# kevalmorabia97/CoVA-Web-Object-Detection

Hardware: AMD Instinct MI355X
Metric: webpages/sec fwd+bwd (90 bboxes, K=24) (higher is better)
Workload: dtype f32

## Files before the change

### cova-web-object-detection_amd/csrc/conv_wgrad4.hip

```cpp
#include "mma.h"
#include "options.h"
#include <type_traits>

#ifndef WG4_ABL
#define WG4_ABL 0
#endif

#if defined(__HIP_DEVICE_COMPILE__) && !defined(__gfx950__)
#error "conv_wgrad4.hip is written for gfx950 (160 KB of LDS per workgroup)"
#endif

#ifdef WG4_TRACE
__device__ unsigned long long g_wg4_trace[2 * 4 * 8];
#define WG4_STAMP(slot)                                                                                         \
    do {                                                                                                        \
        if (blockIdx.x == 0 && (wave == 0 || wave == 4) && wg4_k >= 100 && wg4_k < 104 && lane == 0)           \
            g_wg4_trace[((wave >> 2) * 4 + (wg4_k - 100)) * 8 + (slot)] = __builtin_amdgcn_s_memtime();         \
    } while (0)
#else
#define WG4_STAMP(slot) do { } while (0)
#endif

namespace {

namespace wg4 {
constexpr int THREADS = 512;
constexpr int ROW = 10;
constexpr int TILE_FLOATS = 128 * ROW + 32;
constexpr int BUF_FLOATS = 2 * 4 * TILE_FLOATS;
constexpr int RAW_FLOATS = 36 * 64;
constexpr int PART_FLOATS = 9 * 4096;
}

struct Wg4Args {
    const float *act, *dz, *dz2;
    float *part;
    const float *act_abc, *dz_abc;
    float *dz_out;
    int act_relu;
    int H, W, tiles_y, strips, nseg_y, seg_rows, nsegs;
};

__device__ __forceinline__ void wg4_bt6(const float (&d)[6], float (&o)[6])
{
    const float a = fmaf(-4.f, d[2], d[4]), b = fmaf(-4.f, d[1], d[3]);
    const float c = d[4] - d[2], e = 2.f * (d[3] - d[1]);
    o[0] = fmaf(4.f, d[0], fmaf(-5.f, d[2], d[4]));
    o[1] = a + b;
    o[2] = a - b;
    o[3] = c + e;
    o[4] = c - e;
    o[5] = fmaf(4.f, d[1], fmaf(-5.f, d[3], d[5]));
}

__device__ __forceinline__ void wg4_a6(const float (&g)[4], float (&o)[6])
{
    const float p = g[0] + g[2], q = g[1] + g[3];
    const float u = fmaf(4.f, g[2], g[0]), w = 2.f * fmaf(4.f, g[3], g[1]);
    o[0] = g[0];
    o[1] = p + q;
    o[2] = p - q;
    o[3] = u + w;
    o[4] = u - w;
    o[5] = g[3];
}

template <int HALF>
__device__ __forceinline__ void wg4_bt_half(float d0, float d1, float d2, float d3, float d4, float d5, float (&o)[3])
{
    if (HALF == 0) {
        const float a = fmaf(-4.f, d2, d4), b = fmaf(-4.f, d1, d3);
        o[0] = fmaf(4.f, d0, fmaf(-5.f, d2, d4));
        o[1] = a + b;
        o[2] = a - b;
    } else {
        const float c = d4 - d2, e = 2.f * (d3 - d1);
        o[0] = fmaf(4.f, d1, fmaf(-5.f, d3, d5));
        o[1] = c + e;
        o[2] = c - e;
    }
}

template <int HALF>
__device__ __forceinline__ void wg4_a_half(float g0, float g1, float g2, float g3, float (&o)[3])
{
    if (HALF == 0) {
        const float p = g0 + g2, q = g1 + g3;
        o[0] = g0;
        o[1] = p + q;
        o[2] = p - q;
    } else {
        const float u = fmaf(4.f, g2, g0), w = 2.f * fmaf(4.f, g3, g1);
        o[0] = g3;
        o[1] = u + w;
        o[2] = u - w;
    }
}

struct Wg4It {
    int seg, rr, nrows, b, strip, ty;
};

template <bool PROA, int PROD>
__global__ __launch_bounds__(wg4::THREADS, 1) void conv3x3_wgrad4_kernel(const Wg4Args a)
{
    using namespace wg4;
    __shared__ __attribute__((aligned(16))) float s_op[2 * BUF_FLOATS];
    __shared__ __attribute__((aligned(1024))) float s_raw[8 * RAW_FLOATS];
    const int tid = threadIdx.x, lane = tid & 63;
    const int wave = __builtin_amdgcn_readfirstlane(tid >> 6);
    const int H = a.H, W = a.W;
    const int G = (int)gridDim.x, NW = G >> 1;
    int half, walker;
    if ((G & 15) == 0) {
        const int m = (int)blockIdx.x >> 3, x = (int)blockIdx.x & 7;
        half = m & 1;
        walker = (m >> 1) * 8 + x;
    } else {
        half = (int)blockIdx.x & 1;
        walker = (int)blockIdx.x >> 1;
    }
    const bool vrole = wave < 4;
    const int tcol = wave & 3;
    const int pg = wave & 1, cp = (wave >> 1) & 1, np = wave >> 2;
    const int l15 = lane & 15, kq = lane >> 4;

    int n_k = 0;
    for (int s = walker; s < a.nsegs; s += NW) n_k += min(a.seg_rows, a.tiles_y - (s % a.nseg_y) * a.seg_rows);

    auto seg_setup = [&](Wg4It &it) __attribute__((always_inline)) {
        const int s = it.seg < a.nsegs ? it.seg : walker;
        const int sy = s % a.nseg_y, st = (s / a.nseg_y) % a.strips;
        it.b = s / (a.nseg_y * a.strips);
        it.strip = st;
        it.ty = sy * a.seg_rows;
        it.nrows = min(a.seg_rows, a.tiles_y - it.ty);
        it.rr = 0;
    };
    auto advance = [&](Wg4It &it) __attribute__((always_inline)) {
        if (++it.rr < it.nrows) {
            ++it.ty;
        } else {
            it.seg += NW;
            seg_setup(it);
        }
    };

    f32x4 acc[9][4];
#pragma unroll
    for (int q = 0; q < 9; ++q)
#pragma unroll
        for (int e = 0; e < 4; ++e) acc[q][e] = f32x4{0.f, 0.f, 0.f, 0.f};

    const int a_off = (pg * 4 + kq) * TILE_FLOATS + (32 * cp + l15) * ROW;
    const int b_off = (pg * 4 + kq) * TILE_FLOATS + (64 + 32 * np + l15) * ROW;
    auto mfma_phase = [&](const float *buf) __attribute__((always_inline)) {
        if (WG4_ABL & 1) return;
        const float *pa = (WG4_ABL & 16) ? s_op + a_off : buf + a_off, *pb = (WG4_ABL & 16) ? s_op + b_off : buf + b_off;
        auto pair = [&](const float *p, float (&d)[2]) __attribute__((always_inline)) {
            const float2 v = *reinterpret_cast<const float2 *>(p);
            d[0] = v.x; d[1] = v.y;
        };
#pragma unroll
        for (int q0 = 0; q0 < 8; q0 += 2) {
            float a0[2], a1[2], b0[2], b1[2];
            pair(pa + q0, a0);
            pair(pa + 16 * ROW + q0, a1);
            pair(pb + q0, b0);
            pair(pb + 16 * ROW + q0, b1);
#pragma unroll
            for (int q = 0; q < 2; ++q) {
                acc[q0 + q][0] = mfma16x4(a0[q], b0[q], acc[q0 + q][0]);
                acc[q0 + q][1] = mfma16x4(a0[q], b1[q], acc[q0 + q][1]);
                acc[q0 + q][2] = mfma16x4(a1[q], b0[q], acc[q0 + q][2]);
                acc[q0 + q][3] = mfma16x4(a1[q], b1[q], acc[q0 + q][3]);
            }
        }
        const float a0 = pa[8], a1 = pa[16 * ROW + 8], b0 = pb[8], b1 = pb[16 * ROW + 8];
        acc[8][0] = mfma16x4(a0, b0, acc[8][0]);
        acc[8][1] = mfma16x4(a0, b1, acc[8][1]);
        acc[8][2] = mfma16x4(a1, b0, acc[8][2]);
        acc[8][3] = mfma16x4(a1, b1, acc[8][3]);
    };

    auto run = [&](auto role, auto hsel) __attribute__((always_inline)) {
        constexpr bool VROLE = decltype(role)::value;
        constexpr int HALF = decltype(hsel)::value;
        constexpr int NR = VROLE ? 6 : 4;
        constexpr int NB = NR / 2;
        constexpr bool TWO = !VROLE && PROD == 2;
        const float relu_floor = a.act_relu ? 0.f : -INFINITY;
        float pA = 1.f, pB = 0.f, pC = 0.f;
        if (VROLE) {
            if (PROA) { pA = a.act_abc[lane]; pC = a.act_abc[128 + lane]; }
        } else {
            if (PROD) { pA = a.dz_abc[lane]; pC = a.dz_abc[128 + lane]; }
            if (PROD == 2) pB = a.dz_abc[64 + lane];
        }
        const int sub = lane >> 4, c4 = lane & 15;
        const unsigned laneoff = (unsigned)((((sub >> 1) * W + (sub & 1)) * 64 + c4 * 4) * 4);
        float *raw = s_raw + wave * RAW_FLOATS;
        const unsigned raw_lds = (unsigned)(size_t)(lds_void *)raw;
        const float *raw_r = raw + lane;
        auto range_mask = [&](int g0, int n) __attribute__((always_inline)) {
            const int lo = max(-g0, 0), hi = min(n - g0, NR);
            return hi > lo ? (((1u << hi) - 1u) & ~((1u << lo) - 1u)) : 0u;
        };
        auto masks = [&](const Wg4It &it, unsigned &rm, unsigned &cm) __attribute__((always_inline)) {
            rm = range_mask(4 * it.ty - (VROLE ? 1 : 0), H);
            cm = range_mask(16 * it.strip + 4 * tcol - (VROLE ? 1 : 0), W);
        };
        constexpr unsigned FULL = (1u << NR) - 1u;
        auto piece = [&](const Wg4It &it_, bool edge, int phi, int br, int bc) __attribute__((always_inline)) {
            if (WG4_ABL & 2) return;
            Wg4It it = it_;
            if (WG4_ABL & 32) { it.seg = walker; seg_setup(it); }
            const int gy0 = 4 * it.ty - (VROLE ? 1 : 0), gx0 = 16 * it.strip + 4 * tcol - (VROLE ? 1 : 0);
            const size_t pgb = (size_t)it.b * (size_t)H * (size_t)W * 256u;
            const char *src = reinterpret_cast<const char *>(VROLE ? a.act : a.dz) + pgb;
            const char *src2 = TWO ? reinterpret_cast<const char *>(a.dz2) + pgb : nullptr;
            int ps = br + phi;
            if (VROLE && ps >= 3) ps -= 3;
            const unsigned dst = raw_lds + (VROLE ? 3072u * (unsigned)ps : 2048u * (unsigned)br) + 1024u * (unsigned)bc;
            if (!edge) {
                const unsigned off = (unsigned)(((gy0 + 2 * br) * W + gx0) * 256 + 512 * bc);
                copy16_to_lds(src + off, laneoff, dst);
                if (TWO) copy16_to_lds(src2 + off, laneoff, dst + 4096);
            } else {
                const int r = 2 * br + (sub >> 1), c = 2 * bc + (sub & 1);
                const int gy = min(max(gy0 + r, 0), H - 1), gx = min(max(gx0 + c, 0), W - 1);
                const unsigned eo = (unsigned)((gy * W + gx) * 256 + c4 * 16);
                copy16_to_lds(src, eo, dst);
                if (TWO) copy16_to_lds(src2, eo, dst + 4096);
            }
        };
        auto first_pair = [&](const Wg4It &it) __attribute__((always_inline)) {
            return (VROLE && it.rr != 0 && !(WG4_ABL & 128)) ? 1 : 0;
        };
        auto fetch = [&](const Wg4It &it, bool edge, int phi) __attribute__((always_inline)) {
            const int br0 = first_pair(it);
#pragma unroll
            for (int br = 0; br < NB; ++br) {
                if (br < br0) continue;
#pragma unroll
                for (int bc = 0; bc < NB; ++bc) piece(it, edge, phi, br, bc);
            }
        };
        const bool emit = !VROLE && PROD != 0 && a.dz_out != nullptr;
        int emit_k = 0;
        unsigned emit_lane = (unsigned)lane * 4u;
        asm volatile("" : "+v"(emit_lane));
        unsigned cur_org = 0;
        char *cur_out = reinterpret_cast<char *>(a.dz_out);
        auto origin = [&](const Wg4It &it) __attribute__((always_inline)) {
            cur_out = reinterpret_cast<char *>(a.dz_out) + (size_t)it.b * (size_t)H * (size_t)W * 256u;
            return (unsigned)(((4 * it.ty) * W + 16 * it.strip + 4 * tcol) * 64);
        };
        int phi = 0;
        int wg4_k = -1;
        (void)wg4_k;
        auto transform = [&](float *buf, const Wg4It &nxt, unsigned crm, unsigned ccm, unsigned nrm, unsigned ncm) __attribute__((always_inline)) {
            const float *pair_r[3];
#pragma unroll
            for (int p = 0; p < 3; ++p) {
                int ps = p + phi;
                if (ps >= 3) ps -= 3;
                pair_r[p] = raw_r + (VROLE ? 768 * ps : 512 * p);
            }
            asm volatile("s_waitcnt vmcnt(0)" ::: "memory");
            const int nphi = (!VROLE || (WG4_ABL & 128)) ? 0 : (nxt.rr == 0 ? phi : (phi == 0 ? 2 : phi - 1));
            const bool nedge = nrm != FULL || ncm != FULL;
            if (WG4_ABL & 8) { fetch(nxt, nedge, nphi); phi = nphi; return; }
            WG4_STAMP(1);
            float t[3][NR];
            const bool emit_now = emit && ((emit_k & 1) == HALF);
            ++emit_k;
            auto stage1 = [&](auto cedge_t) __attribute__((always_inline)) {
            constexpr bool cedge = decltype(cedge_t)::value;
#pragma unroll
            for (int c = 0; c < NR; ++c) {
                float d[NR];
#pragma unroll
                for (int r = 0; r < NR; ++r) {
                    const int slot = 4 * (c >> 1) + 2 * (r & 1) + (c & 1);
                    float v = pair_r[r >> 1][64 * slot];
                    if (VROLE && PROA) v = fmaxf(fmaf(pA, v, pC), relu_floor);
                    if (TWO) v = fmaf(pA, v, fmaf(pB, pair_r[r >> 1][64 * (16 + slot)], pC));
                    if (!VROLE && PROD == 1) v = fmaf(pA, v, pC);
                    if (cedge && !(((crm >> r) & (ccm >> c) & 1u) != 0u)) v = 0.f;
                    d[r] = v;
                    if (!VROLE && PROD != 0) {
                        if (emit_now && (!cedge || (((crm >> r) & (ccm >> c) & 1u) != 0u))) {
                            unsigned ob = (cur_org + (unsigned)((r * W + c) * 64)) * 4u;
                            asm volatile("" : "+s"(ob));
                            *reinterpret_cast<float *>(cur_out + ob + emit_lane) = v;
                        }
                    }
                }
                float o[3];
                if constexpr (VROLE) wg4_bt_half<HALF>(d[0], d[1], d[2], d[3], d[4], d[5], o);
                else wg4_a_half<HALF>(d[0], d[1], d[2], d[3], o);
                t[0][c] = o[0]; t[1][c] = o[1]; t[2][c] = o[2];
            }
            };
            if (crm != FULL || ccm != FULL) stage1(std::true_type{});
            else stage1(std::false_type{});
            asm volatile("s_waitcnt lgkmcnt(0)" ::: "memory");
            WG4_STAMP(2);
            fetch(nxt, nedge, nphi);
            phi = nphi;
            WG4_STAMP(3);
            float *r0 = buf + tcol * TILE_FLOATS + ((VROLE ? 64 : 0) + lane) * ROW;
            float *r1 = r0 + 4 * TILE_FLOATS;
#pragma unroll
            for (int al = 0; al < 3; ++al) {
                float o[6];
                if constexpr (VROLE) wg4_bt6(t[al], o);
                else wg4_a6(t[al], o);
                if (al == 0) {
                    *reinterpret_cast<float2 *>(r0) = make_float2(o[0], o[1]);
                    *reinterpret_cast<float2 *>(r0 + 2) = make_float2(o[2], o[3]);
                    *reinterpret_cast<float2 *>(r0 + 4) = make_float2(o[4], o[5]);
                } else if (al == 1) {
                    *reinterpret_cast<float2 *>(r0 + 6) = make_float2(o[0], o[1]);
                    r0[8] = o[2];
                    *reinterpret_cast<float2 *>(r1) = make_float2(o[3], o[4]);
                    r1[2] = o[5];
                } else {
                    r1[3] = o[0];
                    *reinterpret_cast<float2 *>(r1 + 4) = make_float2(o[1], o[2]);
                    *reinterpret_cast<float2 *>(r1 + 6) = make_float2(o[3], o[4]);
                    r1[8] = o[5];
                }
            }
        };

        Wg4It nxt;
        nxt.seg = walker;
        seg_setup(nxt);
        unsigned crm, ccm, nrm, ncm;
        masks(nxt, nrm, ncm);
        fetch(nxt, true, 0);
        crm = nrm; ccm = ncm;
        cur_org = origin(nxt);
        advance(nxt);
        masks(nxt, nrm, ncm);
        transform(s_op, nxt, crm, ccm, nrm, ncm);
        crm = nrm; ccm = ncm;
        cur_org = origin(nxt);
        advance(nxt);
        lds_barrier();
#pragma unroll 1
        for (int k = 0; k < n_k; ++k) {
            wg4_k = k;
            WG4_STAMP(0);
            if (!VROLE || (WG4_ABL & 64)) { mfma_phase(s_op + (k & 1) * BUF_FLOATS); WG4_STAMP(5); }
            const bool more = k + 1 < n_k;
            if (more) {
                masks(nxt, nrm, ncm);
                transform(s_op + ((k + 1) & 1) * BUF_FLOATS, nxt, crm, ccm, nrm, ncm);
            }
            WG4_STAMP(4);
            if (VROLE && !(WG4_ABL & 64)) { mfma_phase(s_op + (k & 1) * BUF_FLOATS); WG4_STAMP(5); }
            if (more) {
                crm = nrm; ccm = ncm;
                cur_org = origin(nxt);
                advance(nxt);
            }
            lds_barrier();
            WG4_STAMP(6);
        }
        asm volatile("s_waitcnt vmcnt(0)" ::: "memory");
    };

    if (n_k > 0) {
        using T = std::true_type;
        using Fl = std::false_type;
        using H0 = std::integral_constant<int, 0>;
        using H1 = std::integral_constant<int, 1>;
        if (vrole) {
            if (half == 0) run(T{}, H0{});
            else run(T{}, H1{});
        } else {
            if (half == 0) run(Fl{}, H0{});
            else run(Fl{}, H1{});
        }
    }
    auto fold_values = [&](auto hsel, auto psel, auto esel, float (&tv)[4][9]) __attribute__((always_inline)) {
        constexpr int HALF = decltype(hsel)::value, PG = decltype(psel)::value, e = decltype(esel)::value;
        constexpr double G[6][3] = {{0.25, 0.0, 0.0},         {-1.0 / 6, -1.0 / 6, -1.0 / 6}, {-1.0 / 6, 1.0 / 6, -1.0 / 6},
                                    {1.0 / 24, 1.0 / 12, 1.0 / 6}, {1.0 / 24, -1.0 / 12, 1.0 / 6}, {0.0, 0.0, 1.0}};
        {
            {
#pragma unroll
            for (int r = 0; r < 4; ++r) {
                double T[9];
#pragma unroll
                for (int k = 0; k < 9; ++k) T[k] = 0.0;
#pragma unroll
                for (int al = 0; al < 3; ++al) {
                    constexpr int p0 = 9 * PG, p1 = 9 * PG + 9;
                    if (6 * al + 6 <= p0 || 6 * al >= p1) continue;
                    const int arow = HALF == 0 ? al : (al == 0 ? 5 : 2 + al);
                    double c[3] = {0.0, 0.0, 0.0};
#pragma unroll
                    for (int b = 0; b < 6; ++b) {
                        const int pos = 6 * al + b;
                        if (pos < p0 || pos >= p1) continue;
                        const double qv = (double)acc[pos - p0][e][r];
#pragma unroll
                        for (int t = 0; t < 3; ++t)
                            if (G[b][t] != 0.0) c[t] = fma(G[b][t], qv, c[t]);
                    }
#pragma unroll
                    for (int r3 = 0; r3 < 3; ++r3)
#pragma unroll
                        for (int t = 0; t < 3; ++t)
                            if (G[arow][r3] != 0.0) T[r3 * 3 + t] = fma(G[arow][r3], c[t], T[r3 * 3 + t]);
                }
#pragma unroll
                for (int k = 0; k < 9; ++k) tv[r][k] = (float)T[k];
            }
            }
        }
    };
    float *dst = a.part + (size_t)blockIdx.x * PART_FLOATS;
    auto fold_round = [&](auto esel) __attribute__((always_inline)) {
        constexpr int e = decltype(esel)::value;
        using H0 = std::integral_constant<int, 0>;
        using H1 = std::integral_constant<int, 1>;
        float *xch = s_op + (e & 1) * (4 * 36 * 64) + (wave >> 1) * (36 * 64) + lane;
        float tv[4][9];
        if (half == 0) { if (pg == 0) fold_values(H0{}, H0{}, esel, tv); else fold_values(H0{}, H1{}, esel, tv); }
        else           { if (pg == 0) fold_values(H1{}, H0{}, esel, tv); else fold_values(H1{}, H1{}, esel, tv); }
        if (pg == 1) {
#pragma unroll
            for (int r = 0; r < 4; ++r)
#pragma unroll
                for (int k = 0; k < 9; ++k) xch[(r * 9 + k) * 64] = tv[r][k];
        }
        __syncthreads();
        if (pg == 0) {
            const int i = e >> 1, j = e & 1;
#pragma unroll
            for (int r = 0; r < 4; ++r)
#pragma unroll
                for (int k = 0; k < 9; ++k)
                    dst[k * 4096 + (16 * (2 * cp + i) + 4 * kq + r) * 64 + 16 * (2 * np + j) + l15] =
                        tv[r][k] + xch[(r * 9 + k) * 64];
        }
    };
    __syncthreads();
    fold_round(std::integral_constant<int, 0>{});
    fold_round(std::integral_constant<int, 1>{});
    fold_round(std::integral_constant<int, 2>{});
    fold_round(std::integral_constant<int, 3>{});
}

struct Wg4FinishJobs { const float *part[4]; float *dw[4]; };
__global__ __launch_bounds__(1024) void wgrad4_finish_kernel(const Wg4FinishJobs jobs, int grid)
{
    __shared__ double s_acc[9][16][64];
    const float *__restrict__ part = jobs.part[blockIdx.y];
    float *__restrict__ dw = jobs.dw[blockIdx.y];
    const int tx = threadIdx.x & 63, slice = threadIdx.x >> 6;
    const int idx = blockIdx.x * 64 + tx;
    double acc[9];
#pragma unroll
    for (int k = 0; k < 9; ++k) acc[k] = 0.0;
    for (int blk0 = slice; blk0 < grid; blk0 += 16 * 8) {
        float v[8][9];
#pragma unroll
        for (int u = 0; u < 8; ++u) {
            const int blk = blk0 + 16 * u;
            const float *row = part + (size_t)(blk < grid ? blk : blk0) * wg4::PART_FLOATS + idx;
#pragma unroll
            for (int k = 0; k < 9; ++k) v[u][k] = row[k * 4096];
        }
#pragma unroll
        for (int u = 0; u < 8; ++u)
            if (blk0 + 16 * u < grid) {
#pragma unroll
                for (int k = 0; k < 9; ++k) acc[k] += (double)v[u][k];
            }
    }
#pragma unroll
    for (int k = 0; k < 9; ++k) s_acc[k][slice][tx] = acc[k];
    __syncthreads();
    if (slice < 9) {
        double t = 0.0;
        for (int j = 0; j < 16; ++j) t += s_acc[slice][j][tx];
        dw[idx * 9 + slice] = (float)t;
    }
}

struct Wg4Geo { int tiles_y, strips, nseg_y, seg_rows, nsegs, grid; };

Wg4Geo wg4_geometry(int B, int H, int W)
{
    Wg4Geo g;
    g.tiles_y = cdiv(H, 4);
    g.strips = cdiv(W, 16);
    g.nseg_y = (g.tiles_y + 10) / 20 > 0 ? (g.tiles_y + 10) / 20 : 1;
    g.seg_rows = cdiv(g.tiles_y, g.nseg_y);
    g.nseg_y = cdiv(g.tiles_y, g.seg_rows);
    g.nsegs = B * g.strips * g.nseg_y;
    const int cus = cova_internal_persistent_grid2(1 << 30, 1);
    int walkers = cus / 2 > 0 ? cus / 2 : 1;
    if (walkers > g.nsegs) walkers = g.nsegs;
    g.grid = 2 * walkers;
    return g;
}

int launch_wgrad4(const float *act, const float *act_abc, int act_relu, const float *dz, const float *dz2,
                  const float *dz_abc, float *dz_out, float *ws, int B, int H, int W, hipStream_t st)
{
    const Wg4Geo g = wg4_geometry(B, H, W);
    const Wg4Args a{act, dz, dz_abc ? dz2 : nullptr, ws, act_abc, dz_abc, dz_abc ? dz_out : nullptr, act_relu, H, W,
                    g.tiles_y, g.strips, g.nseg_y, g.seg_rows, g.nsegs};
    const dim3 grid(g.grid), blk(wg4::THREADS);
    const int prod = !dz_abc ? 0 : (dz2 ? 2 : 1);
#define COVA_WG4(PA, PD) hipLaunchKernelGGL((conv3x3_wgrad4_kernel<PA, PD>), grid, blk, 0, st, a)
    if (act_abc) { if (prod == 2) COVA_WG4(true, 2); else if (prod == 1) COVA_WG4(true, 1); else COVA_WG4(true, 0); }
    else         { if (prod == 2) COVA_WG4(false, 2); else if (prod == 1) COVA_WG4(false, 1); else COVA_WG4(false, 0); }
#undef COVA_WG4
    COVA_LAUNCH_CHECK();
    return COVA_OK;
}

}

COVA_API int cova_conv3x3_wgrad4_num_partials(int B, int H, int W) { return wg4_geometry(B, H, W).grid; }

COVA_API int cova_conv3x3_wgrad4_workspace_floats(int B, int H, int W)
{
    const int grid = wg4_geometry(B, H, W).grid;
    return grid * wg4::PART_FLOATS;
}

COVA_API int cova_conv3x3_wgrad4_partial(const float *act, const float *act_abc, int act_relu, const float *dz,
                                         const float *dz2, const float *dz_abc, float *dz_out, float *ws, int B, int H,
                                         int W, void *stream)
{
    COVA_REQUIRE(act && dz && ws && B > 0 && H > 0 && W > 0);
    COVA_REQUIRE((long long)H * W * 256 < (1ll << 32));
    COVA_REQUIRE(dz_out == nullptr || dz_abc != nullptr);
    return launch_wgrad4(act, act_abc, act_relu, dz, dz2, dz_abc, dz_out, ws, B, H, W, (hipStream_t)stream);
}

COVA_API int cova_conv3x3_wgrad4_finish(const float *ws0, float *dw0, const float *ws1, float *dw1, const float *ws2,
                                        float *dw2, const float *ws3, float *dw3, int B, int H, int W, void *stream)
{
    COVA_REQUIRE(B > 0 && H > 0 && W > 0);
    COVA_REQUIRE((ws0 == nullptr) == (dw0 == nullptr) && (ws1 == nullptr) == (dw1 == nullptr) &&
                 (ws2 == nullptr) == (dw2 == nullptr) && (ws3 == nullptr) == (dw3 == nullptr));
    const float *ws[4] = {ws0, ws1, ws2, ws3};
    float *dw[4] = {dw0, dw1, dw2, dw3};
    Wg4FinishJobs jobs{};
    int n = 0;
    for (int i = 0; i < 4; ++i)
        if (ws[i]) { jobs.part[n] = ws[i]; jobs.dw[n] = dw[i]; ++n; }
    if (n == 0) return COVA_OK;
    const int grid = wg4_geometry(B, H, W).grid;
    hipLaunchKernelGGL(wgrad4_finish_kernel, dim3(4096 / 64, n), dim3(1024), 0, (hipStream_t)stream, jobs, grid);
    COVA_LAUNCH_CHECK();
    return COVA_OK;
}

#ifdef WG4_TRACE
COVA_API int cova_wg4_trace_read(unsigned long long *host64)
{
    return (int)hipMemcpyFromSymbol(host64, HIP_SYMBOL(g_wg4_trace), sizeof(unsigned long long) * 64);
}
#endif

COVA_API int cova_conv3x3_wgrad4(const float *act, const float *dz, float *dw, float *ws, int B, int H, int W, void *stream)
{
    COVA_REQUIRE(act && dz && dw && ws && B > 0 && H > 0 && W > 0);
    const int rc = launch_wgrad4(act, nullptr, 0, dz, nullptr, nullptr, nullptr, ws, B, H, W, (hipStream_t)stream);
    if (rc != COVA_OK) return rc;
    return cova_conv3x3_wgrad4_finish(ws, dw, nullptr, nullptr, nullptr, nullptr, nullptr, nullptr, B, H, W, stream);
}
```

### cova-web-object-detection_amd/csrc/mma.h

```cpp
#pragma once
#include "bf3.h"

__device__ __forceinline__ f32x4 mfma16x4(float a, float b, f32x4 c)
{
    return __builtin_amdgcn_mfma_f32_16x16x4f32(a, b, c, 0, 0, 0);
}

__device__ __forceinline__ f32x16 mfma32bf(u32x4 a, u32x4 b, f32x16 c)
{
    return __builtin_amdgcn_mfma_f32_32x32x16_bf16(__builtin_bit_cast(bf16x8, a), __builtin_bit_cast(bf16x8, b), c, 0, 0, 0);
}

typedef __attribute__((address_space(3))) void lds_void;

__device__ __forceinline__ void copy16_to_lds(const void *base, unsigned off_bytes, unsigned lds_base_bytes)
{
    asm volatile("s_mov_b32 m0, %0\n\tglobal_load_lds_dwordx4 %1, %2" ::"s"(lds_base_bytes), "v"(off_bytes), "s"(base) : "memory", "m0");
}

__device__ __forceinline__ void lds_barrier() { asm volatile("s_waitcnt lgkmcnt(0)\n\ts_barrier" ::: "memory"); }
```

Measured before the change: 1749.

## Specialize wgrad4 transform for interior tiles and precompute walk addresses

Reworks the Winograd weight-gradient kernel's tile walker so it carries precomputed source, output and origin addresses plus a column mask, advancing incrementally rather than recomputing per tile. Interior tiles get a compile-time specialized transform with no mask checks and batched side-output stores. Loads and stores use immediate offsets, kernel arguments are reloaded from the kernarg segment to reduce register pressure, and the LDS pair rotation becomes pointer rotation. This aims to cut scalar/vector address arithmetic and register use in the hot loop, at the cost of extra code-size from more template instantiations.

Measured after the change: 1814 (median of 6 runs). +3.7%, better.

```diff
diff --git a/cova-web-object-detection_amd/csrc/conv_wgrad4.hip b/cova-web-object-detection_amd/csrc/conv_wgrad4.hip
--- a/cova-web-object-detection_amd/csrc/conv_wgrad4.hip
+++ b/cova-web-object-detection_amd/csrc/conv_wgrad4.hip
@@ -4,6 +4,12 @@
 
 #ifndef WG4_ABL
 #define WG4_ABL 0
+#endif
+#if WG4_ABL & (32 | 128)
+#error "WG4_ABL masks 32 and 128 are retired"
+#endif
+#ifndef WG4_SERIAL_READS
+#define WG4_SERIAL_READS 0
 #endif
 
 #if defined(__HIP_DEVICE_COMPILE__) && !defined(__gfx950__)
@@ -40,6 +46,14 @@
     int act_relu;
     int H, W, tiles_y, strips, nseg_y, seg_rows, nsegs;
 };
+
+typedef __attribute__((address_space(4))) const Wg4Args wg4_kernarg;
+__device__ __forceinline__ wg4_kernarg *wg4_kernarg_fresh()
+{
+    wg4_kernarg *p = reinterpret_cast<wg4_kernarg *>(reinterpret_cast<size_t>(__builtin_amdgcn_kernarg_segment_ptr()));
+    asm volatile("" : "+s"(p));
+    return p;
+}
 
 __device__ __forceinline__ void wg4_bt6(const float (&d)[6], float (&o)[6])
 {
@@ -97,9 +111,40 @@
     }
 }
 
-struct Wg4It {
-    int seg, rr, nrows, b, strip, ty;
+struct Wg4Walk {
+    int seg, rr, nrows, ty;
+    int gx0;
+    unsigned cm;
+    unsigned org;
+    const char *src, *src2;
+    char *out;
 };
+
+template <int I, int N, class F>
+__device__ __forceinline__ void wg4_for(F &&f)
+{
+    if constexpr (I < N) {
+        f(std::integral_constant<int, I>{});
+        wg4_for<I + 1, N>(f);
+    }
+}
+
+__device__ __forceinline__ float wg4_lds_read(unsigned byte_addr)
+{
+    typedef __attribute__((address_space(3))) const float lds_cfloat;
+    float v = *reinterpret_cast<lds_cfloat *>((size_t)byte_addr);
+#if WG4_SERIAL_READS
+    asm volatile("" : "+v"(v) : : "memory");
+#endif
+    return v;
+}
+
+template <int IMM>
+__device__ __forceinline__ void wg4_store_imm(char *base, unsigned off_bytes, float v)
+{
+    static_assert(IMM >= 0 && IMM < 4096, "global_store: 13-bit signed immediate offset");
+    asm volatile("global_store_dword %0, %1, %2 offset:%3" ::"v"(off_bytes), "v"(v), "s"(base), "i"(IMM));
+}
 
 template <bool PROA, int PROD>
 __global__ __launch_bounds__(wg4::THREADS, 1) void conv3x3_wgrad4_kernel(const Wg4Args a)
@@ -128,24 +173,6 @@
     int n_k = 0;
     for (int s = walker; s < a.nsegs; s += NW) n_k += min(a.seg_rows, a.tiles_y - (s % a.nseg_y) * a.seg_rows);
 
-    auto seg_setup = [&](Wg4It &it) __attribute__((always_inline)) {
-        const int s = it.seg < a.nsegs ? it.seg : walker;
-        const int sy = s % a.nseg_y, st = (s / a.nseg_y) % a.strips;
-        it.b = s / (a.nseg_y * a.strips);
-        it.strip = st;
-        it.ty = sy * a.seg_rows;
-        it.nrows = min(a.seg_rows, a.tiles_y - it.ty);
-        it.rr = 0;
-    };
-    auto advance = [&](Wg4It &it) __attribute__((always_inline)) {
-        if (++it.rr < it.nrows) {
-            ++it.ty;
-        } else {
-            it.seg += NW;
-            seg_setup(it);
-        }
-    };
-
     f32x4 acc[9][4];
 #pragma unroll
     for (int q = 0; q < 9; ++q)
@@ -189,6 +216,8 @@
         constexpr int NR = VROLE ? 6 : 4;
         constexpr int NB = NR / 2;
         constexpr bool TWO = !VROLE && PROD == 2;
+        constexpr int V = VROLE ? 1 : 0;
+        constexpr bool SIDE = !VROLE && PROD != 0;
         const float relu_floor = a.act_relu ? 0.f : -INFINITY;
         float pA = 1.f, pB = 0.f, pC = 0.f;
         if (VROLE) {
@@ -198,117 +227,158 @@
             if (PROD == 2) pB = a.dz_abc[64 + lane];
         }
         const int sub = lane >> 4, c4 = lane & 15;
+        const unsigned W256 = (unsigned)W * 256u;
         const unsigned laneoff = (unsigned)((((sub >> 1) * W + (sub & 1)) * 64 + c4 * 4) * 4);
-        float *raw = s_raw + wave * RAW_FLOATS;
-        const unsigned raw_lds = (unsigned)(size_t)(lds_void *)raw;
-        const float *raw_r = raw + lane;
+        unsigned rowoff[NB];
+#pragma unroll
+        for (int br = 0; br < NB; ++br) rowoff[br] = laneoff + 2u * (unsigned)br * W256;
+        const unsigned raw_lds = (unsigned)(size_t)(lds_void *)(s_raw + wave * RAW_FLOATS);
+        const unsigned lane4 = (unsigned)lane * 4u;
         auto range_mask = [&](int g0, int n) __attribute__((always_inline)) {
             const int lo = max(-g0, 0), hi = min(n - g0, NR);
             return hi > lo ? (((1u << hi) - 1u) & ~((1u << lo) - 1u)) : 0u;
         };
-        auto masks = [&](const Wg4It &it, unsigned &rm, unsigned &cm) __attribute__((always_inline)) {
-            rm = range_mask(4 * it.ty - (VROLE ? 1 : 0), H);
-            cm = range_mask(16 * it.strip + 4 * tcol - (VROLE ? 1 : 0), W);
-        };
         constexpr unsigned FULL = (1u << NR) - 1u;
-        auto piece = [&](const Wg4It &it_, bool edge, int phi, int br, int bc) __attribute__((always_inline)) {
+        auto seg_setup = [&](Wg4Walk &w) __attribute__((always_inline)) {
+            wg4_kernarg *ka = wg4_kernarg_fresh();
+            const int nsegs = ka->nsegs, nseg_y = ka->nseg_y, strips = ka->strips, seg_rows = ka->seg_rows, tiles_y = ka->tiles_y;
+            const int s = w.seg < nsegs ? w.seg : walker;
+            const int q = s / nseg_y, sy = s - q * nseg_y;
+            const int b = q / strips, st = q - b * strips;
+            w.ty = sy * seg_rows;
+            w.nrows = min(seg_rows, tiles_y - w.ty);
+            w.rr = 0;
+            w.gx0 = 16 * st + 4 * tcol - V;
+            w.cm = range_mask(w.gx0, W);
+            w.org = (unsigned)(((4 * w.ty - V) * W + w.gx0) * 256);
+            const size_t pgb = (size_t)b * (size_t)H * (size_t)W * 256u;
+            w.src = reinterpret_cast<const char *>(VROLE ? ka->act : ka->dz) + pgb;
+            w.src2 = TWO ? reinterpret_cast<const char *>(ka->dz2) + pgb : nullptr;
+            w.out = SIDE ? reinterpret_cast<char *>(ka->dz_out) + pgb : nullptr;
+        };
+        auto advance = [&](Wg4Walk &w) __attribute__((always_inline)) {
+            if (++w.rr < w.nrows) {
+                ++w.ty;
+                w.org += 4u * W256;
+            } else {
+                w.seg += NW;
+                seg_setup(w);
+            }
+        };
+        auto is_edge = [&](const Wg4Walk &w) __attribute__((always_inline)) {
+            return w.cm != FULL || w.ty < V || 4 * w.ty - V + NR > H;
+        };
+        unsigned pb[3] = {raw_lds, raw_lds + (VROLE ? 3072u : 2048u), raw_lds + (VROLE ? 6144u : 4096u)};
+        auto fetch_in = [&](const Wg4Walk &w, const unsigned (&nb)[3], int br0) __attribute__((always_inline)) {
             if (WG4_ABL & 2) return;
-            Wg4It it = it_;
-            if (WG4_ABL & 32) { it.seg = walker; seg_setup(it); }
-            const int gy0 = 4 * it.ty - (VROLE ? 1 : 0), gx0 = 16 * it.strip + 4 * tcol - (VROLE ? 1 : 0);
-            const size_t pgb = (size_t)it.b * (size_t)H * (size_t)W * 256u;
-            const char *src = reinterpret_cast<const char *>(VROLE ? a.act : a.dz) + pgb;
-            const char *src2 = TWO ? reinterpret_cast<const char *>(a.dz2) + pgb : nullptr;
-            int ps = br + phi;
-            if (VROLE && ps >= 3) ps -= 3;
-            const unsigned dst = raw_lds + (VROLE ? 3072u * (unsigned)ps : 2048u * (unsigned)br) + 1024u * (unsigned)bc;
-            if (!edge) {
-                const unsigned off = (unsigned)(((gy0 + 2 * br) * W + gx0) * 256 + 512 * bc);
-                copy16_to_lds(src + off, laneoff, dst);
-                if (TWO) copy16_to_lds(src2 + off, laneoff, dst + 4096);
-            } else {
-                const int r = 2 * br + (sub >> 1), c = 2 * bc + (sub & 1);
-                const int gy = min(max(gy0 + r, 0), H - 1), gx = min(max(gx0 + c, 0), W - 1);
-                const unsigned eo = (unsigned)((gy * W + gx) * 256 + c4 * 16);
-                copy16_to_lds(src, eo, dst);
-                if (TWO) copy16_to_lds(src2, eo, dst + 4096);
-            }
-        };
-        auto first_pair = [&](const Wg4It &it) __attribute__((always_inline)) {
-            return (VROLE && it.rr != 0 && !(WG4_ABL & 128)) ? 1 : 0;
-        };
-        auto fetch = [&](const Wg4It &it, bool edge, int phi) __attribute__((always_inline)) {
-            const int br0 = first_pair(it);
+            const char *p = w.src + w.org;
+            const char *p2 = TWO ? w.src2 + w.org : nullptr;
+            wg4_for<0, NB>([&](auto br_t) __attribute__((always_inline)) {
+                constexpr int br = decltype(br_t)::value;
+                if (br < br0) return;
+                wg4_for<0, NB>([&](auto bc_t) __attribute__((always_inline)) {
+                    constexpr int bc = decltype(bc_t)::value;
+                    const unsigned base = VROLE ? nb[br] : raw_lds;
+                    constexpr int add = (VROLE ? 0 : 2048 * br) + 512 * bc;
+                    copy16_to_lds_imm<512 * bc, add>(p, rowoff[br], base);
+                    if (TWO) copy16_to_lds_imm<512 * bc, add + 4096>(p2, rowoff[br], base);
+                });
+            });
+        };
+        auto fetch_edge = [&](const Wg4Walk &w, const unsigned (&nb)[3], int br0) __attribute__((always_inline)) {
+            if (WG4_ABL & 2) return;
+            const int gy0 = 4 * w.ty - V;
 #pragma unroll
             for (int br = 0; br < NB; ++br) {
                 if (br < br0) continue;
 #pragma unroll
-                for (int bc = 0; bc < NB; ++bc) piece(it, edge, phi, br, bc);
-            }
-        };
-        const bool emit = !VROLE && PROD != 0 && a.dz_out != nullptr;
+                for (int bc = 0; bc < NB; ++bc) {
+                    const unsigned dst = nb[br] + 1024u * (unsigned)bc;
+                    const int r = 2 * br + (sub >> 1), c = 2 * bc + (sub & 1);
+                    const int gy = min(max(gy0 + r, 0), H - 1), gx = min(max(w.gx0 + c, 0), W - 1);
+                    const unsigned eo = (unsigned)((gy * W + gx) * 256 + c4 * 16);
+                    copy16_to_lds(w.src, eo, dst);
+                    if (TWO) copy16_to_lds(w.src2, eo, dst + 4096);
+                }
+            }
+        };
+        const bool emit = SIDE && a.dz_out != nullptr;
         int emit_k = 0;
-        unsigned emit_lane = (unsigned)lane * 4u;
-        asm volatile("" : "+v"(emit_lane));
-        unsigned cur_org = 0;
-        char *cur_out = reinterpret_cast<char *>(a.dz_out);
-        auto origin = [&](const Wg4It &it) __attribute__((always_inline)) {
-            cur_out = reinterpret_cast<char *>(a.dz_out) + (size_t)it.b * (size_t)H * (size_t)W * 256u;
-            return (unsigned)(((4 * it.ty) * W + 16 * it.strip + 4 * tcol) * 64);
-        };
-        int phi = 0;
+        unsigned outoff[4];
+#pragma unroll
+        for (int r = 0; r < 4; ++r) outoff[r] = lane4 + (unsigned)r * W256;
+        bool cur_edge = true;
+        int cur_ty = 0;
+        unsigned cur_cm = 0, cur_org = 0;
+        char *cur_out = nullptr;
         int wg4_k = -1;
         (void)wg4_k;
-        auto transform = [&](float *buf, const Wg4It &nxt, unsigned crm, unsigned ccm, unsigned nrm, unsigned ncm) __attribute__((always_inline)) {
-            const float *pair_r[3];
-#pragma unroll
-            for (int p = 0; p < 3; ++p) {
-                int ps = p + phi;
-                if (ps >= 3) ps -= 3;
-                pair_r[p] = raw_r + (VROLE ? 768 * ps : 512 * p);
-            }
+        auto transform = [&](float *buf, const Wg4Walk &nxt, auto interior_t, auto emit_t, bool emit_rt) __attribute__((always_inline)) {
+            constexpr bool INTERIOR = decltype(interior_t)::value;
+            constexpr bool EMIT = decltype(emit_t)::value;
             asm volatile("s_waitcnt vmcnt(0)" ::: "memory");
-            const int nphi = (!VROLE || (WG4_ABL & 128)) ? 0 : (nxt.rr == 0 ? phi : (phi == 0 ? 2 : phi - 1));
-            const bool nedge = nrm != FULL || ncm != FULL;
-            if (WG4_ABL & 8) { fetch(nxt, nedge, nphi); phi = nphi; return; }
+            const bool down = INTERIOR || nxt.rr != 0;
+            unsigned nb[3] = {pb[0], pb[1], pb[2]};
+            if (VROLE && down) { nb[0] = pb[2]; nb[1] = pb[0]; nb[2] = pb[1]; }
+            const int br0 = (VROLE && down) ? 1 : 0;
+            auto fetch = [&]() __attribute__((always_inline)) {
+                if constexpr (INTERIOR) {
+                    fetch_in(nxt, nb, VROLE ? 1 : 0);
+                } else {
+                    if (is_edge(nxt)) fetch_edge(nxt, nb, br0);
+                    else fetch_in(nxt, nb, br0);
+                }
+#pragma unroll
+                for (int p = 0; p < 3; ++p) pb[p] = nb[p];
+            };
+            if (WG4_ABL & 8) { fetch(); return; }
             WG4_STAMP(1);
             float t[3][NR];
-            const bool emit_now = emit && ((emit_k & 1) == HALF);
-            ++emit_k;
-            auto stage1 = [&](auto cedge_t) __attribute__((always_inline)) {
-            constexpr bool cedge = decltype(cedge_t)::value;
-#pragma unroll
-            for (int c = 0; c < NR; ++c) {
+            unsigned crm = FULL, ccm = FULL;
+            if (!INTERIOR) { crm = range_mask(4 * cur_ty - V, H); ccm = cur_cm; }
+            unsigned ra[3];
+#pragma unroll
+            for (int p = 0; p < NB; ++p) ra[p] = pb[p] + lane4;
+            char *obase = SIDE ? cur_out + cur_org : nullptr;
+            float keep[SIDE && INTERIOR && EMIT ? 4 : 1][4];
+            (void)keep;
+            wg4_for<0, NR>([&](auto c_t) __attribute__((always_inline)) {
+                constexpr int c = decltype(c_t)::value;
                 float d[NR];
-#pragma unroll
-                for (int r = 0; r < NR; ++r) {
-                    const int slot = 4 * (c >> 1) + 2 * (r & 1) + (c & 1);
-                    float v = pair_r[r >> 1][64 * slot];
+                wg4_for<0, NR>([&](auto r_t) __attribute__((always_inline)) {
+                    constexpr int r = decltype(r_t)::value;
+                    constexpr int slot = 4 * (c >> 1) + 2 * (r & 1) + (c & 1);
+                    float v = wg4_lds_read(ra[r >> 1] + 256u * slot);
                     if (VROLE && PROA) v = fmaxf(fmaf(pA, v, pC), relu_floor);
-                    if (TWO) v = fmaf(pA, v, fmaf(pB, pair_r[r >> 1][64 * (16 + slot)], pC));
+                    if (TWO) v = fmaf(pA, v, fmaf(pB, wg4_lds_read(ra[r >> 1] + 256u * (16 + slot)), pC));
                     if (!VROLE && PROD == 1) v = fmaf(pA, v, pC);
-                    if (cedge && !(((crm >> r) & (ccm >> c) & 1u) != 0u)) v = 0.f;
+                    const bool inside = INTERIOR || (((crm >> r) & (ccm >> c) & 1u) != 0u);
+                    if (!inside) v = 0.f;
                     d[r] = v;
-                    if (!VROLE && PROD != 0) {
-                        if (emit_now && (!cedge || (((crm >> r) & (ccm >> c) & 1u) != 0u))) {
-                            unsigned ob = (cur_org + (unsigned)((r * W + c) * 64)) * 4u;
-                            asm volatile("" : "+s"(ob));
-                            *reinterpret_cast<float *>(cur_out + ob + emit_lane) = v;
+                    if constexpr (SIDE) {
+                        if constexpr (INTERIOR) {
+                            if constexpr (EMIT) keep[c][r] = v;
+                        } else {
+                            if (emit_rt && inside) wg4_store_imm<256 * c>(obase, outoff[r], v);
                         }
                     }
-                }
+                });
                 float o[3];
                 if constexpr (VROLE) wg4_bt_half<HALF>(d[0], d[1], d[2], d[3], d[4], d[5], o);
                 else wg4_a_half<HALF>(d[0], d[1], d[2], d[3], o);
                 t[0][c] = o[0]; t[1][c] = o[1]; t[2][c] = o[2];
-            }
-            };
-            if (crm != FULL || ccm != FULL) stage1(std::true_type{});
-            else stage1(std::false_type{});
+            });
+            if constexpr (SIDE && INTERIOR && EMIT) {
+                wg4_for<0, 4>([&](auto c_t) __attribute__((always_inline)) {
+                    wg4_for<0, 4>([&](auto r_t) __attribute__((always_inline)) {
+                        constexpr int c = decltype(c_t)::value, r = decltype(r_t)::value;
+                        wg4_store_imm<256 * c>(obase, outoff[r], keep[c][r]);
+                    });
+                });
+            }
             asm volatile("s_waitcnt lgkmcnt(0)" ::: "memory");
             WG4_STAMP(2);
-            fetch(nxt, nedge, nphi);
-            phi = nphi;
+            fetch();
             WG4_STAMP(3);
             float *r0 = buf + tcol * TILE_FLOATS + ((VROLE ? 64 : 0) + lane) * ROW;
             float *r1 = r0 + 4 * TILE_FLOATS;
@@ -335,20 +405,28 @@
             }
         };
 
-        Wg4It nxt;
+        using Tt = std::true_type;
+        using Ft = std::false_type;
+        Wg4Walk nxt;
         nxt.seg = walker;
         seg_setup(nxt);
-        unsigned crm, ccm, nrm, ncm;
-        masks(nxt, nrm, ncm);
-        fetch(nxt, true, 0);
-        crm = nrm; ccm = ncm;
-        cur_org = origin(nxt);
-        advance(nxt);
-        masks(nxt, nrm, ncm);
-        transform(s_op, nxt, crm, ccm, nrm, ncm);
-        crm = nrm; ccm = ncm;
-        cur_org = origin(nxt);
-        advance(nxt);
+        auto step_walk = [&]() __attribute__((always_inline)) {
+            cur_edge = is_edge(nxt);
+            cur_ty = nxt.ty;
+            cur_cm = nxt.cm;
+            cur_org = nxt.org;
+            cur_out = nxt.out;
+            advance(nxt);
+        };
+        auto my_turn = [&]() __attribute__((always_inline)) {
+            const bool now = emit && ((emit_k & 1) == HALF);
+            ++emit_k;
+            return now;
+        };
+        fetch_edge(nxt, pb, 0);
+        step_walk();
+        transform(s_op, nxt, Ft{}, Ft{}, my_turn());
+        step_walk();
         lds_barrier();
 #pragma unroll 1
         for (int k = 0; k < n_k; ++k) {
@@ -357,16 +435,19 @@
             if (!VROLE || (WG4_ABL & 64)) { mfma_phase(s_op + (k & 1) * BUF_FLOATS); WG4_STAMP(5); }
             const bool more = k + 1 < n_k;
             if (more) {
-                masks(nxt, nrm, ncm);
-                transform(s_op + ((k + 1) & 1) * BUF_FLOATS, nxt, crm, ccm, nrm, ncm);
+                float *nbuf = s_op + ((k + 1) & 1) * BUF_FLOATS;
+                const bool turn = my_turn();
+                const bool interior = !cur_edge && !is_edge(nxt) && !(VROLE && nxt.rr == 0);
+                if (interior) {
+                    if (SIDE && turn) transform(nbuf, nxt, Tt{}, Tt{}, true);
+                    else transform(nbuf, nxt, Tt{}, Ft{}, false);
+                } else {
+                    transform(nbuf, nxt, Ft{}, Ft{}, turn);
+                }
             }
             WG4_STAMP(4);
             if (VROLE && !(WG4_ABL & 64)) { mfma_phase(s_op + (k & 1) * BUF_FLOATS); WG4_STAMP(5); }
-            if (more) {
-                crm = nrm; ccm = ncm;
-                cur_org = origin(nxt);
-                advance(nxt);
-            }
+            if (more) step_walk();
             lds_barrier();
             WG4_STAMP(6);
         }
@@ -424,7 +505,7 @@
             }
         }
     };
-    float *dst = a.part + (size_t)blockIdx.x * PART_FLOATS;
+    float *dst = wg4_kernarg_fresh()->part + (size_t)blockIdx.x * PART_FLOATS;
     auto fold_round = [&](auto esel) __attribute__((always_inline)) {
         constexpr int e = decltype(esel)::value;
         using H0 = std::integral_constant<int, 0>;
diff --git a/cova-web-object-detection_amd/csrc/mma.h b/cova-web-object-detection_amd/csrc/mma.h
--- a/cova-web-object-detection_amd/csrc/mma.h
+++ b/cova-web-object-detection_amd/csrc/mma.h
@@ -18,4 +18,15 @@
     asm volatile("s_mov_b32 m0, %0\n\tglobal_load_lds_dwordx4 %1, %2" ::"s"(lds_base_bytes), "v"(off_bytes), "s"(base) : "memory", "m0");
 }
 
+template <int IMM, int LDS_ADD>
+__device__ __forceinline__ void copy16_to_lds_imm(const void *base, unsigned off_bytes, unsigned lds_base_bytes)
+{
+    static_assert(IMM >= 0 && IMM < 4096, "global_load_lds: 13-bit signed immediate offset");
+    static_assert(LDS_ADD >= 0 && LDS_ADD < 65536, "LDS byte offset");
+    if constexpr (LDS_ADD == 0)
+        asm volatile("s_mov_b32 m0, %0\n\tglobal_load_lds_dwordx4 %1, %2 offset:%3" ::"s"(lds_base_bytes), "v"(off_bytes), "s"(base), "i"(IMM) : "memory", "m0");
+    else
+        asm volatile("s_add_u32 m0, %0, %4\n\tglobal_load_lds_dwordx4 %1, %2 offset:%3" ::"s"(lds_base_bytes), "v"(off_bytes), "s"(base), "i"(IMM), "i"(LDS_ADD) : "memory", "m0", "scc");
+}
+
 __device__ __forceinline__ void lds_barrier() { asm volatile("s_waitcnt lgkmcnt(0)\n\ts_barrier" ::: "memory"); }
```
